# smoorjani/matrix-multiplication

Hardware: AMD Instinct MI355X
Metric: SpMM GFLOP/s, CSR(1M,0.01%) x dense(256) (higher is better)
Workload: dtype f32

## Files before the change

### include/mi_spmm.h

```cpp
#ifndef MI_SPMM_H_
#define MI_SPMM_H_

#include <stddef.h>
#include <stdint.h>

#ifdef __cplusplus
extern "C" {
#endif

#define MI_SPMM_ABI_VERSION 1

typedef void* mi_stream_t;

enum {
  MI_OK = 0,
  MI_EINVAL = -1,
  MI_ERANGE = -2,
  MI_EHIP = -3,
  MI_ENOMEM = -4,
  MI_EUNSORTED = -5
};

int mi_spmm_abi_version(void);
const char* mi_status_string(int status);
// ... 31 lines not shown
  MI_SPMM_GROUP_VEC4 = 4,
  MI_SPMM_GROUP_SCALAR = 5,
  MI_SPMM_WAVE_ROW_VL = 6,
  MI_SPMM_PANELS_2 = 7,
  MI_SPMM_PANELS_3 = 8,
  MI_SPMM_PANELS_4 = 9,
  MI_SPMM_PANELS_5 = 10,
  MI_SPMM_PANELS_6 = 11,
  MI_SPMM_PANELS_8 = 12,
  MI_SPMM_GROUP_VEC2 = 13,
  MI_SPMM_COLTILE = 14,
  MI_SPMM_COLTILE_PANELS = 15,
  MI_SPMM_NARROW = 16,
  MI_SPMM_SLAB = 17,
  MI_SPMM_LDS_B = 18,
  MI_SPMM_GROUP_PANELS_2 = 19,
  MI_SPMM_GROUP_PANELS_3 = 20,
  MI_SPMM_GROUP_PANELS_4 = 21,
  MI_SPMM_GROUP_PANELS_6 = 22,
  MI_SPMM_GROUP_PANELS_8 = 23,
  MI_SPMM_GROUP_VEC4U = 24,
  MI_SPMM_VARIANT_COUNT = 25
};
int mi_spmm_ldsb_set_form(int form);
int mi_spmm_csr_f32_variant(int variant, const int32_t* rowptr, const int32_t* col,
                            const float* val, int64_t nnz, int32_t M, int32_t K,
                            int32_t N, const float* B, int64_t ldb, float* C,
                            int64_t ldc, mi_stream_t stream);
int mi_spmm_csr_ex_variant_f32(int variant, const int32_t* rowptr, const int32_t* col, const float* val,
                               int64_t nnz, int32_t M, int32_t K, int32_t N, const float* B, int64_t ldb,
                               const float* bias, float* C, int64_t ldc, int long_rows, void* workspace,
                               size_t workspace_bytes, mi_stream_t stream);

int mi_spmm_csr_f32_plan(int64_t nnz, int32_t M, int32_t K, int32_t N, const float* B,
                         int64_t ldb, const float* C, int64_t ldc);
int mi_spmm_variant_launches(int variant);
const char* mi_spmm_variant_name(int variant);

typedef struct mi_spmm_schedule mi_spmm_schedule_t;
size_t mi_spmm_schedule_workspace_bytes(int32_t M);
#define MI_SCHEDULE_HOST_INTS 512
int mi_spmm_schedule_begin(const int32_t* rowptr, const int32_t* col, int32_t M, int32_t K, int64_t nnz, int32_t N,
                           int32_t* order, int32_t* order_locality, void* workspace, size_t workspace_bytes,
                           int32_t* host_out, mi_stream_t stream);
int mi_spmm_schedule_finish(const int32_t* host_out, int32_t* order, int32_t* order_locality, int32_t M, int32_t K, int64_t nnz,
                            int32_t N, mi_spmm_schedule_t** out);
int mi_spmm_schedule_create(const int32_t* rowptr, const int32_t* col, int32_t M, int32_t K, int64_t nnz, int32_t N,
                            int32_t* order, void* workspace, size_t workspace_bytes, mi_stream_t stream,
                            mi_spmm_schedule_t** out);
int mi_spmm_schedule_destroy(mi_spmm_schedule_t* schedule);
#define MI_SPMM_SCHEDULE_INFO_LEN 12
int mi_spmm_schedule_info(const mi_spmm_schedule_t* schedule, int64_t* info);
int mi_spmm_schedule_set_heavy(mi_spmm_schedule_t* schedule, int32_t heavy_len, int use_side_stream);
int mi_spmm_csr_scheduled_f32(const mi_spmm_schedule_t* schedule, int variant, const int32_t* rowptr, const int32_t* col,
                              const float* val, int64_t nnz, int32_t M, int32_t K, int32_t N, const float* B, int64_t ldb,
                              const float* bias, float* C, int64_t ldc, int long_rows, void* workspace,
                              size_t workspace_bytes, mi_stream_t stream);
int mi_spmm_csr_colmajor_sched_f32(const mi_spmm_schedule_t* schedule, const int32_t* rowptr, const int32_t* col,
                                   const float* val, int64_t nnz, int32_t M, int32_t K, int32_t N, const float* B,
                                   int64_t ldb, float* C, int64_t ldc, int long_rows, void* long_rows_workspace,
                                   size_t long_rows_workspace_bytes, void* workspace, size_t workspace_bytes,
                                   mi_stream_t stream);

int mi_spmm_csr_batched_f32(const int32_t* rowptr, const int32_t* col,
                            const float* val, int64_t nnz_total, int32_t batch,
                            int32_t M, int32_t K, int32_t N, const float* B,
                            int64_t ldb, int64_t strideB, float* C, int64_t ldc,
                            int64_t strideC, mi_stream_t stream);
int mi_spmm_csr_batched_perm_f32(const int32_t* rowptr, const int32_t* col, const float* val,
                                 const int32_t* perm, int64_t nnz_total, int32_t batch, int32_t M,
                                 int32_t K, int32_t N, const float* B, int64_t ldb, int64_t strideB,
                                 float* C, int64_t ldc, int64_t strideC, mi_stream_t stream);
int mi_spmm_csr_batched_variant_f32(int variant, const int32_t* rowptr, const int32_t* col,
                                    const float* val, int64_t nnz_total, int32_t batch,
                                    int32_t M, int32_t K, int32_t N, const float* B,
                                    int64_t ldb, int64_t strideB, float* C, int64_t ldc,
                                    int64_t strideC, mi_stream_t stream);
int mi_spmm_csr_batched_at_f32(const int32_t* rowptr, const int32_t* col, const float* val, int64_t nnz_total,
                               int32_t batch, int32_t M, int32_t K, int32_t N, const float* X, int64_t ldx,
                               int64_t strideX, float* Y, int64_t ldy, int64_t strideY, mi_stream_t stream);
int mi_batched_csr_narrow_i64(const int64_t* crow, const int64_t* col, int32_t batch, int32_t M, int64_t per_item,
                              int32_t* offsets, int32_t* columns, mi_stream_t stream);
int mi_spmm_csr_batched_f32_plan(int64_t nnz_total, int32_t batch, int32_t M, int32_t K, int32_t N,
                                 const float* B, int64_t ldb, int64_t strideB, const float* C,
                                 int64_t ldc, int64_t strideC);

size_t mi_spmm_colmajor_workspace_bytes(int32_t M, int32_t K, int32_t N);
int mi_spmm_csr_colmajor_f32(const int32_t* rowptr, const int32_t* col,
                             const float* val, int64_t nnz, int32_t M, int32_t K,
                             int32_t N, const float* B, int64_t ldb, float* C,
                             int64_t ldc, void* workspace, size_t workspace_bytes,
                             mi_stream_t stream);
int mi_spmm_colmajor_native_form(int64_t nnz, int32_t M, int32_t K, int32_t N, const float* B,
                                 int64_t ldb, const float* C, int64_t ldc);
int mi_spmm_colmajor_form(int64_t nnz, int32_t M, int32_t K, int32_t N, const float* B, int64_t ldb,
                          const float* C, int64_t ldc, const void* workspace);
int mi_spmm_csr_colmajor_ex_f32(const int32_t* rowptr, const int32_t* col,
                                const float* val, int64_t nnz, int32_t M, int32_t K,
                                int32_t N, const float* B, int64_t ldb, float* C,
                                int64_t ldc, int long_rows, void* long_rows_workspace,
                                size_t long_rows_workspace_bytes, void* workspace,
                                size_t workspace_bytes, mi_stream_t stream);

int mi_gemm_f32(int transa, int transb, int32_t m, int32_t n, int32_t k,
                const float* A, int64_t lda, int64_t strideA, const float* B,
                int64_t ldb, int64_t strideB, float* C, int64_t ldc,
// ... 137 lines not shown
```

### matrix-multiplication_amd/csrc/custom_mm.cpp

```cpp
#include <torch/extension.h>

#include <c10/hip/HIPGuard.h>
#include <c10/hip/HIPStream.h>

#include <array>
#include <cstdlib>
#include <initializer_list>
#include <map>
#include <memory>
#include <mutex>
#include <string>
#include <tuple>
#include <unordered_map>
#include <utility>

#include "mi_spmm.h"

namespace {
#include "custom_mm_helpers.inc"
#include "custom_mm_reference.inc"
#include "custom_mm_extras.inc"
#include "custom_mm_inspect.inc"
#include "custom_mm_reduce.inc"

// ... 32 lines not shown
  m.def("cusparse_mmul", &cusparse_mmul, "cuSPARSE Torch Matrix Multiplication");

  m.def("dummy_kernel", &dummy_kernel_launch, "Launch dummy kernel.");
  m.def("naive_spmm", &naive_spmm, "A naive implementation of Sparse Matrix Multiplication");

  m.def("tiledspmm_inspect_csr", &tiledspmm_inspect_csr, "Inspect function for TiledSpMM with CSR input");
  m.def("tiledspmm_inspect_coo", &tiledspmm_inspect_coo, "Inspect function for TiledSpMM with COO input");
  m.def("tiledspmm_mm", &tiledspmm_mm, "MM function for TiledSpMM");
  m.def("tiledspmm_clean", &tiledspmm_clean, "Cleanup function for TiledSpMM");

  m.def("cusparse_inspect", &cusparse_inspect, "Inspect function for CuSPARSE with CSR input");
  m.def("cusparse_mmul_opt", &cusparse_mmul_opt, "MM function for CuSPARSE");
  m.def("cusparse_clean", &cusparse_clean, "Cleanup function for CuSPARSE");
  m.def("cusparse_mmul_opt_t", &cusparse_mmul_opt_t, "column-major product with the cached transpose: C = A^T B");
  m.def("tiledspmm_mm_t", &tiledspmm_mm_t, "column-major product with the cached transpose: C = A^T B");
  m.def("inspect_info", &inspect_info, "what an inspector handle holds (layer, tiled)");

  m.def("dense_to_csr", &dense_to_csr, "Device dense -> batched CSR (values, columns, offsets)");
  m.def("dense_row_offsets", &dense_row_offsets, "Device dense -> row offsets [batch, rows+1] only (no host sync)");
  m.def("dense_to_csr_fill", &dense_to_csr_fill, "(values, columns) for the offsets of dense_row_offsets");
  m.def("naive_spmm_batched", &naive_spmm_batched, "Batched CSR x dense in one launch");
  m.def("csr_transpose", &csr_transpose, "Device CSR transpose (values, columns, offsets)");
  m.def("csr_transpose_batched", &csr_transpose_batched, "Batched device CSR transpose (values, columns, offsets [batch, cols+1])");
  m.def("csr_transpose_in_lds", [](int64_t nnz, int64_t batch, int64_t rows, int64_t cols) {
          return rows <= INT32_MAX && cols <= INT32_MAX && batch <= INT32_MAX &&
                 mi_csr_transpose_batched_in_lds(nnz, (int32_t)batch, (int32_t)rows, (int32_t)cols) == 1;
        }, "does csr_transpose_batched run the one-workgroup-per-item LDS plan on this batch (cheap: transpose per backward)");
  m.def("sddmm", &sddmm, "Sampled dense-dense product on a CSR pattern");
  m.def("cublas_bmm_pair", &cublas_bmm_pair,
        "dA = dC.B and dB = dC^T.A in one launch that reads dC once; (dC, B, A, dA, dB) -> launched?");
  m.def("sddmm_batched", &sddmm_batched,
        "SDDMM on a batched CSR pattern into out[nnz]; False (nothing launched) if the LDS-resident form does not take it");
  m.def("gather_perm", &gather_perm, "values[perm] (int32 perm) as a new tensor");
  m.def("naive_spmm_batched_perm", &naive_spmm_batched_perm,
        "naive_spmm_batched with entry p's value = A_values[perm[p]]; False (nothing launched) if the plan takes no permutation");
  m.def("naive_spmm_batched_at", &naive_spmm_batched_at,
        "C[i] = A[i]^T X[i] for a batched CSR A without transposing it; False (nothing launched) if the shape is not covered");
  m.def("batched_csr_narrow", &batched_csr_narrow,
        "(int32 offsets [batch, rows+1] with the items' bases, int32 columns) of int64 crow [batch, rows+1] / col [batch, per_item]");
  m.def("naive_spmm_dense", &naive_spmm_dense,
        "A·B with A dense, zeros skipped in the kernel; False if the shape is not covered");
  m.def("naive_spmm_dense_bias", &naive_spmm_dense_bias, "as naive_spmm_dense, + bias in the epilogue");
  m.def("nonfinite_flag", &nonfinite_flag, "int32[1] device tensor: 1 if the tensor holds an inf / nan (nothing read back)");
  m.def("naive_spmm_dense_gated", &naive_spmm_dense_gated,
        "naive_spmm_dense as a launch that runs only when flag[0] != 0 on the device; (A, B, C, flag, dry_run) -> covered?");
  m.def("cublas_mmul_bias", &cublas_mmul_bias, "op(A) op(B) + bias, fused epilogue");
  m.def("column_sums", &column_sums, "sum over rows of a 2-d tensor (bias gradient)");
  m.def("naive_spmm_bias", &naive_spmm_bias, "CSR x dense + bias, fused epilogue");
  m.def("naive_spmm_ex", &naive_spmm_ex, "naive_spmm with the long-row rule pinned (-1 auto, 0 none, 1 split)");
  m.def("naive_spmm_bias_ex", &naive_spmm_bias_ex, "naive_spmm_bias with the long-row rule pinned (-1 auto, 0 none, 1 split)");
  m.def("spmm_plan", &spmm_plan, "(variant, kernel name, launches, splits_long_rows) of the AUTO plan");
  m.def("validate_csr", &validate_csr, "opt-in check of CSR contents (offsets monotone, columns in range); raises");
  py::class_<PySchedule, std::shared_ptr<PySchedule>>(m, "SpmmSchedule")
      .def("info", &PySchedule::info, "rows, heavy_rows, heavy_length, classes, longest_at_least, side_stream, active, locality_order, window spans, nnz, width")
      .def("set_heavy", &PySchedule::set_heavy, py::arg("heavy_length"), py::arg("side_stream") = true,
           "another heavy length / the heavy launch in line (tests, A/B)")
      .def_readonly("order", &PySchedule::order, "int32 [rows] on the device: slot -> row, rows by descending length class");
  m.def("spmm_schedule", &spmm_schedule, py::arg("A_offsets"), py::arg("nnzA"), py::arg("A_rows"), py::arg("N"),
        py::arg("A_columns") = py::none(), py::arg("A_cols") = 0,
        "Inspector: the row schedule of a CSR matrix (offsets, nnz, rows, dense width; with the columns: also tries the locality order)");
  m.def("naive_spmm_scheduled", &naive_spmm_scheduled, py::arg("schedule"), py::arg("A_values"), py::arg("A_columns"),
        py::arg("A_offsets"), py::arg("nnzA"), py::arg("A_rows"), py::arg("A_cols"), py::arg("B"), py::arg("C"),
        py::arg("bias") = py::none(), py::arg("long_rows") = -1, py::arg("variant") = 0,
        "naive_spmm on a row schedule: the same bits, rows handed to waves longest first");
  m.def("auto_schedule_stats", &auto_schedule_stats, "the automatic row schedules of the plain entry points: enabled, entries, pending, active, inactive, built");
  m.def("auto_schedule_clear", &auto_schedule_clear, "forget every automatic row schedule");
  m.def("ipc_export", &ipc_export, "(handle bytes, offset, allocation bytes) of a device buffer, for a peer process to map");
  m.def("ipc_open", &ipc_open, "a peer's exported buffer as a tensor (valid until ipc_close of the handle)");
  m.def("ipc_close", &ipc_close, "drop one open of a peer handle");
  m.def("ipc_open_count", []() { return mi_ipc_open_count(); }, "peer mappings not yet closed in this process");
  m.def("long_row_threshold", &long_row_threshold, "rows with more non-zeros are 'long' (split rule)");
  m.def("naive_spmm_reduce", &naive_spmm_reduce, py::arg("A_values"), py::arg("A_columns"), py::arg("A_offsets"),
        py::arg("nnzA"), py::arg("A_rows"), py::arg("A_cols"), py::arg("B"), py::arg("C"), py::arg("reduce"),
        py::arg("arg") = py::none(),
        "CSR x dense with reduce = sum / mean / amax / amin (torch.sparse.mm); amax / amin write the selected entries to arg");
  m.def("spmm_rows_divide", &spmm_rows_divide, "out = in / (entries of the row), per row (mean and its gradient)");
  m.def("spmm_reduce_grad_val", &spmm_reduce_grad_val, "amax / amin: gradient of A's stored values from the forward's arg");
  m.def("spmm_reduce_grad_b", &spmm_reduce_grad_b, "amax / amin: gradient of B on A^T's pattern and permutation");
  py::module_::import("atexit").attr("register")(py::cpp_function([]() {
    auto_schedule_clear();
    std::lock_guard<std::mutex> lock(g_registry_mutex);
    g_cusparse_layers.clear();
    g_tiled_layers.clear();
  }));
}
```

### matrix-multiplication_amd/csrc/custom_mm_reference.inc

```

torch::Tensor cublas_mmul(torch::Tensor A, torch::Tensor B, torch::Tensor C, bool transa,
                          bool transb) {
  return gemm_impl(A, B, C, 0, transa, transb, "cublas_mmul");
}

torch::Tensor cublas_bmm(torch::Tensor A, torch::Tensor B, torch::Tensor C, int dim, bool transa,
                         bool transb) {
  if (dim == 3) return gemm_impl(A, B, C, 1, transa, transb, "cublas_bmm");
  if (dim == 4) return gemm_impl(A, B, C, 2, transa, transb, "cublas_bmm");
  if (dim == 2) return cublas_mmul(A, B, C, transa, transb);
  throw std::invalid_argument("Invalid dim argument.");
}


struct StreamWorkspace {
  torch::Tensor buf;
};
std::mutex g_stream_ws_mutex;
std::map<std::pair<int, mi_stream_t>, StreamWorkspace> g_stream_ws;

bool stream_is_capturing(mi_stream_t stream) {
  hipStreamCaptureStatus status = hipStreamCaptureStatusNone;
  if (hipStreamIsCapturing(static_cast<hipStream_t>(stream), &status) != hipSuccess) {
    (void)hipGetLastError();
    return true;
  }
  return status != hipStreamCaptureStatusNone;
}

torch::Tensor zeroed_stream_workspace(const torch::Device& dev, mi_stream_t stream, size_t bytes) {
  std::lock_guard<std::mutex> lock(g_stream_ws_mutex);
  const auto key = std::make_pair((int)dev.index(), stream);
  if (g_stream_ws.size() >= 64 && g_stream_ws.find(key) == g_stream_ws.end())
    g_stream_ws.clear();
  StreamWorkspace& w = g_stream_ws[key];
  if (!w.buf.defined() || (size_t)w.buf.numel() < bytes) {
    const int64_t cap = (int64_t)(bytes + bytes / 2 + 4096);
    w.buf = torch::empty({cap}, torch::dtype(torch::kUInt8).device(dev));
    w.buf.narrow(0, 0, 16).zero_();
  }
  return w.buf;
}

void drop_stream_workspace(const torch::Device& dev, mi_stream_t stream) {
  std::lock_guard<std::mutex> lock(g_stream_ws_mutex);
  g_stream_ws.erase(std::make_pair((int)dev.index(), stream));
}

std::array<int64_t, MI_SPMM_SCHEDULE_INFO_LEN> schedule_info(const mi_spmm_schedule_t* sc, const char* what) {
  std::array<int64_t, MI_SPMM_SCHEDULE_INFO_LEN> v{};
  check_status(mi_spmm_schedule_info(sc, v.data()), what);
  return v;
}

struct PySchedule {
  torch::Tensor order;
  torch::Tensor order_keep;
  mi_spmm_schedule_t* sc = nullptr;
  int64_t rows = 0, nnz = 0;
  torch::Tensor long_ws;
  int64_t long_ws_width = -1;
  int64_t long_rows = -1;
  ~PySchedule() { mi_spmm_schedule_destroy(sc); }
  py::dict info() const {
    const auto v = schedule_info(sc, "SpmmSchedule.info");
    py::dict d;
    d["rows"] = v[0];
    d["heavy_rows"] = v[1];
    d["heavy_length"] = v[2];
    d["classes"] = v[3];
    d["longest_at_least"] = v[4];
    d["side_stream"] = (v[5] & 1) != 0;
    d["active"] = (v[5] & 2) != 0;
    d["locality_order"] = (v[5] & 4) != 0;
    d["window_span_natural"] = v[8] < 0 ? -1.0 : v[8] / 1000.0;
    d["window_span_scheduled"] = v[9] < 0 ? -1.0 : v[9] / 1000.0;
    d["row_span"] = v[10] < 0 ? -1.0 : v[10] / 1000.0;
    d["long_rows"] = long_rows;
    d["nnz"] = v[6];
    d["width"] = v[7];
    d["long_rows_prepared"] = long_ws.defined();
    return d;
  }
  void set_heavy(int64_t heavy_len, bool side_stream) {
    check_status(mi_spmm_schedule_set_heavy(sc, (int32_t)heavy_len, side_stream ? 1 : 0), "SpmmSchedule.set_heavy");
  }
};

struct AutoEntry {
  int seen = 0;
  bool pending = false, failed = false, active = false;
  std::shared_ptr<PySchedule> sched;
  torch::Tensor order_buf, ws, host;
  hipEvent_t ev = nullptr;
  uint64_t stamp = 0;
};
using AutoKey = std::tuple<int, mi_stream_t, const void*, const void*, int64_t, int64_t>;
std::mutex g_auto_mutex;
std::map<AutoKey, AutoEntry> g_auto;
uint64_t g_auto_clock = 0;
int64_t g_auto_built = 0;

bool auto_schedule_enabled() {
  static const bool on = []() {
    const char* e = std::getenv("MI_AUTO_SCHEDULE");
    return !(e != nullptr && e[0] == '0');
  }();
  return on;
}

void auto_drop(AutoEntry& e) {
  if (e.ev != nullptr) (void)hipEventDestroy(e.ev);
  e.ev = nullptr;
}

std::shared_ptr<PySchedule> auto_schedule(const torch::Tensor& A_offsets, const torch::Tensor& A_columns, int64_t nnzA,
                                          int64_t A_rows, int64_t A_cols, int64_t N, mi_stream_t stream) {
  if (!auto_schedule_enabled() || nnzA < (1 << 14) || A_rows < 1024 || A_cols > INT32_MAX || stream_is_capturing(stream)) return nullptr;
  std::lock_guard<std::mutex> lock(g_auto_mutex);
  const AutoKey key{(int)A_offsets.device().index(), stream, A_offsets.data_ptr(), A_columns.data_ptr(), A_rows, nnzA};
  AutoEntry& e = g_auto[key];
  e.seen++;
  e.stamp = ++g_auto_clock;
  if (e.sched) return e.active ? e.sched : nullptr;
  if (e.failed) return nullptr;
  if (e.pending) {
    if (e.ev == nullptr) return nullptr;
    const hipError_t q = hipEventQuery(e.ev);
    if (q == hipErrorNotReady) {
      (void)hipGetLastError();
      return nullptr;
    }
    e.pending = false;
    auto_drop(e);
    if (q != hipSuccess) {
      e.failed = true;
      return nullptr;
    }
    auto out = std::make_shared<PySchedule>();
    int32_t* order = e.order_buf.data_ptr<int32_t>();
    if (mi_spmm_schedule_finish(e.host.data_ptr<int32_t>(), order, order + A_rows, (int32_t)A_rows, (int32_t)A_cols, nnzA, (int32_t)N,
                                &out->sc) != MI_OK) {
      e.failed = true;
      return nullptr;
    }
    const auto v = schedule_info(out->sc, "auto_schedule");
    out->rows = A_rows;
    out->nnz = nnzA;
    out->order_keep = e.order_buf;
    out->order = (v[5] & 4) ? e.order_buf.narrow(0, A_rows, A_rows) : e.order_buf.narrow(0, 0, A_rows);
    if (!(v[5] & 2)) out->order_keep = out->order = torch::Tensor();
    e.order_buf = e.ws = e.host = torch::Tensor();
    e.sched = out;
    e.active = (v[5] & 2) != 0;
    g_auto_built++;
    return e.active ? e.sched : nullptr;
  }
  if (e.seen == 2) {
    try {
      auto iopt = torch::dtype(torch::kInt32).device(A_offsets.device());
      e.order_buf = torch::empty({2 * A_rows}, iopt);
      e.ws = byte_workspace(A_offsets.device(), mi_spmm_schedule_workspace_bytes((int32_t)A_rows));
      e.host = torch::empty({MI_SCHEDULE_HOST_INTS}, torch::dtype(torch::kInt32).pinned_memory(true));
      e.pending = true;
    } catch (...) {
      e.failed = true;
      e.order_buf = e.ws = e.host = torch::Tensor();
    }
  }
  if (g_auto.size() > 16) {
    auto victim = g_auto.end();
    for (auto it = g_auto.begin(); it != g_auto.end(); ++it)
      if (!it->second.pending && &it->second != &e && (victim == g_auto.end() || it->second.stamp < victim->second.stamp)) victim = it;
    if (victim != g_auto.end()) {
      auto_drop(victim->second);
      g_auto.erase(victim);
    }
  }
  return nullptr;
}

void auto_schedule_launch(const torch::Tensor& A_offsets, const torch::Tensor& A_columns, int64_t nnzA, int64_t A_rows,
                          int64_t A_cols, int64_t N, mi_stream_t stream) {
  if (!auto_schedule_enabled()) return;
  std::lock_guard<std::mutex> lock(g_auto_mutex);
  auto it = g_auto.find(AutoKey{(int)A_offsets.device().index(), stream, A_offsets.data_ptr(), A_columns.data_ptr(), A_rows, nnzA});
  if (it == g_auto.end()) return;
  AutoEntry& e = it->second;
  if (!e.pending || e.ev != nullptr || !e.order_buf.defined()) return;
  int32_t* order = e.order_buf.data_ptr<int32_t>();
  const int st = mi_spmm_schedule_begin(A_offsets.data_ptr<int32_t>(), A_columns.data_ptr<int32_t>(), (int32_t)A_rows, (int32_t)A_cols,
                                        nnzA, (int32_t)N, order, order + A_rows, e.ws.data_ptr(), (size_t)e.ws.numel(),
                                        e.host.data_ptr<int32_t>(), stream);
  bool ok = st == MI_OK && hipEventCreateWithFlags(&e.ev, hipEventDisableTiming) == hipSuccess &&
            hipEventRecord(e.ev, static_cast<hipStream_t>(stream)) == hipSuccess;
  if (!ok) {
    auto_drop(e);
    e.pending = false;
    e.failed = true;
    e.order_buf = e.ws = e.host = torch::Tensor();
  }
}

py::dict auto_schedule_stats() {
  std::lock_guard<std::mutex> lock(g_auto_mutex);
  int64_t pending = 0, active = 0, inactive = 0;
  for (auto& kv : g_auto) {
// ... 250 lines not shown
```

### matrix-multiplication_amd/csrc/spmm_csr.hip

```cpp
#include "spmm_device.h"
#include "spmm_internal.h"

namespace {

using mi::LongArg;
using mi::Shape;

template <int T, int U>
__global__ __launch_bounds__(256) void spmm_wave_row_kernel(
    const int* __restrict__ rowptr, const int* __restrict__ col,
    const float* __restrict__ val, const float* __restrict__ B, float* __restrict__ C,
    int M, long ldb, long ldc, long strideB, long strideC, const float* __restrict__ bias,
    LongArg la) {
  const int lane = threadIdx.x & 63;
  const int wave = __builtin_amdgcn_readfirstlane(threadIdx.x >> 6);
  const long slot = (long)blockIdx.x * 4 + wave;
  if (slot >= (la.order ? la.nslots : M)) return;
  const long row = la.order ? la.order[slot] : slot;
  const long item = blockIdx.y;
  const int* rp = rowptr + item * ((long)M + 1);
  const float* Bl = B + item * strideB + lane * 4;
  float* Cl = C + item * strideC + row * ldc + lane * 4;

  int p = rp[row];
// ... 501 lines not shown
      return dispatch_group<4>(rowptr, col, val, B, C, M, N, ldb, ldc, strideB, strideC, batch, bias, la, s);
    }
    case MI_SPMM_NARROW: {
      if (N >= 4) return MI_EINVAL;
      const long blocks = ((long)M + 3) / 4;
      if (blocks > 0x7fffffffL) return MI_ERANGE;
      hipLaunchKernelGGL(spmm_narrow_kernel, dim3((unsigned)blocks, (unsigned)batch), dim3(256), 0, s, rowptr, col,
                         val, B, C, M, N, ldb, ldc, strideB, strideC, bias);
      return mi::check_launch();
    }
    default:
      return MI_EINVAL;
  }
#undef MI_WAVE
}

bool variant_takes_order(int variant) {
  switch (variant) {
    case MI_SPMM_WAVE_ROW_U4: case MI_SPMM_WAVE_ROW_U8: case MI_SPMM_WAVE_ROW_U16:
    case MI_SPMM_GROUP_VEC4: case MI_SPMM_GROUP_VEC2: case MI_SPMM_GROUP_SCALAR: case MI_SPMM_GROUP_VEC4U:
    case MI_SPMM_PANELS_2: case MI_SPMM_PANELS_3: case MI_SPMM_PANELS_4: case MI_SPMM_PANELS_5: case MI_SPMM_PANELS_6:
    case MI_SPMM_PANELS_8:
    case MI_SPMM_GROUP_PANELS_2: case MI_SPMM_GROUP_PANELS_3: case MI_SPMM_GROUP_PANELS_4: case MI_SPMM_GROUP_PANELS_6:
    case MI_SPMM_GROUP_PANELS_8:
      return true;
    default:
      return false;
  }
}

}

namespace mi {

int spmm_dispatch(int variant, const int32_t* rowptr, const int32_t* col, const float* val,
                  int64_t nnz, int32_t batch, int32_t M, int32_t K, int32_t N, const float* B,
                  int64_t ldb, int64_t strideB, float* C, int64_t ldc, int64_t strideC,
                  const float* bias, void* workspace, size_t workspace_bytes, hipStream_t s,
                  int long_mode, const RowSchedule* sched) {
  if (M < 0 || K < 0 || N < 0 || nnz < 0 || batch < 0) return MI_EINVAL;
  if (variant < 0 || variant >= MI_SPMM_VARIANT_COUNT) return MI_EINVAL;
  if (long_mode < MI_LONG_ROWS_AUTO || long_mode > MI_LONG_ROWS_AUTO_ZEROED) return MI_EINVAL;
  if (nnz > 0x7fffffffLL) return MI_ERANGE;
  if (batch > 65535) return MI_ERANGE;
  if (M == 0 || N == 0 || batch == 0) return MI_OK;
  if (!rowptr || !C) return MI_EINVAL;
  if (nnz > 0 && (!col || !val || !B)) return MI_EINVAL;
  if (ldb < N || ldc < N) return MI_EINVAL;
  if (sched != nullptr && (sched->rows != M || sched->order == nullptr || batch != 1)) return MI_EINVAL;

  Shape sh = classify(N, ldb, ldc, strideB, strideC, B, C);
  if (bias && !mi::aligned16(bias)) sh.vec4_ok = sh.wave_ok = false;
  if (bias && (reinterpret_cast<uintptr_t>(bias) & 7u)) sh.vec2_ok = false;
  if (variant == MI_SPMM_AUTO) variant = choose_variant(sh, nnz, batch, M, K, N, ldb);
  if (sched != nullptr && (!sched->active || !variant_takes_order(variant))) sched = nullptr;

  const bool pinned_split = long_mode == MI_LONG_ROWS_SPLIT || long_mode == MI_LONG_ROWS_PREPARED;
  const bool split = workspace != nullptr && batch == 1 && nnz > kLongRow && variant != MI_SPMM_NARROW &&
                     long_mode != MI_LONG_ROWS_NONE && (variant != MI_SPMM_SLAB || pinned_split);
  int* ws = static_cast<int*>(workspace);
  const LongWs lw = long_ws_layout(nnz, N);
  LongArg la = {0x7fffffff, 0, 0, 0, nullptr, nullptr, nullptr, 0};
  const bool prepared = long_mode == MI_LONG_ROWS_PREPARED;
  const bool panel_plan = (variant >= MI_SPMM_PANELS_2 && variant <= MI_SPMM_PANELS_8) ||
                          (variant >= MI_SPMM_GROUP_PANELS_2 && variant <= MI_SPMM_GROUP_PANELS_8);
  const double b_bytes_all = (double)K * (double)ldb * 4.0;
  if (panel_plan && batch == 1 && nnz > 0 && b_bytes_all < 768.0 * 1048576.0 && workspace != nullptr && workspace_bytes >= lw.bytes &&
      (reinterpret_cast<uintptr_t>(workspace) & 15u) == 0) {
    int* verdicts = reinterpret_cast<int*>(static_cast<char*>(workspace) + lw.adapt_off);
    const int st = launch_locality_probe(rowptr, col, M, ldb, b_bytes_all, verdicts, sched != nullptr ? sched->order : nullptr, s);
    if (st != MI_OK) return st;
    la.adapt = verdicts;
  }
  if (split) {
    if (workspace_bytes < lw.bytes) return MI_ENOMEM;
    if ((reinterpret_cast<uintptr_t>(workspace) & 15u) != 0) return MI_EINVAL;
    la.thresh = kLongRow;
    la.cap_e = (int)lw.cap_e, la.cap_s = (int)lw.cap_s, la.cap_p = (int)lw.cap_p;
    if (!prepared) {
      if (long_mode != MI_LONG_ROWS_AUTO_ZEROED) MI_HIP_TRY(hipMemsetAsync(ws, 0, 16, s));
      if (variant == MI_SPMM_SLAB || variant == MI_SPMM_LDS_B) {
        LongArg fl = la;
        fl.ws = ws;
        const int st = launch_find_long_rows(rowptr, M, fl, s);
        if (st != MI_OK) return st;
      } else {
        la.ws = ws;
      }
    }
  }
  int st = MI_OK;
  bool long_rows_done = false;
  if (sched == nullptr) {
    st = launch_variant(variant, sh, rowptr, col, val, nnz, batch, M, K, N, B, ldb, strideB, C, ldc, strideC, bias, la, s);
  } else {
    const int heavy_slots = sched->heavy < 0 ? 0 : (sched->heavy > M ? M : sched->heavy);
    const int heavy = N >= 4 ? heavy_slots : 0;
    LongArg lh = la, lr = la;
    lh.order = sched->order, lh.nslots = heavy;
    lh.adapt = nullptr;
    const bool early_list = split && !prepared && heavy_slots > 0 && la.ws != nullptr;
    const bool fork = sched->side != nullptr && sched->fork != nullptr && sched->join != nullptr &&
                      (heavy > 0 || (split && prepared) || early_list);
    if (early_list) {
      st = launch_find_long_rows(rowptr, M, la, s);
      if (st != MI_OK) return st;
    }
    hipStream_t rest = s;
    if (fork) {
      MI_HIP_TRY(hipEventRecord(sched->fork, s));
      MI_HIP_TRY(hipStreamWaitEvent(sched->side, sched->fork, 0));
      rest = sched->side;
    }
    if (early_list) {
      lh.ws = nullptr;
      st = launch_staged_rows(ws, lw, false, lh, rowptr, col, val, B, C, N, ldb, ldc, bias, s);
      if (st != MI_OK) return st;
      MI_HIP_TRY(hipMemsetAsync(ws, 0, 16, s));
      long_rows_done = true;
      lr.ws = nullptr;
    } else if (split && prepared && heavy > 0) {
      st = launch_staged_rows(ws, lw, false, lh, rowptr, col, val, B, C, N, ldb, ldc, bias, s);
      if (st != MI_OK) return st;
      long_rows_done = true;
    } else if (split && prepared) {
      st = launch_long_rows(ws, lw, rowptr, col, val, B, C, N, ldb, ldc, bias, false, s);
      if (st != MI_OK) return st;
      long_rows_done = true;
    } else if (heavy > 0) {
      st = launch_heavy_rows(rowptr, col, val, M, N, B, ldb, C, ldc, bias, lh, s);
      if (st != MI_OK) return st;
    }
    lr.order = sched->order + heavy, lr.nslots = M - heavy;
    st = launch_variant(variant, sh, rowptr, col, val, nnz, batch, M, K, N, B, ldb, strideB, C, ldc, strideC, bias, lr, rest);
    if (fork) {
      MI_HIP_TRY(hipEventRecord(sched->join, sched->side));
      MI_HIP_TRY(hipStreamWaitEvent(s, sched->join, 0));
    }
  }
  if (st != MI_OK || !split || long_rows_done) return st;
  return launch_long_rows(ws, lw, rowptr, col, val, B, C, N, ldb, ldc, bias, !prepared, s);
}

}

namespace {
// ... 119 lines not shown
```

### matrix-multiplication_amd/csrc/spmm_internal.h

```cpp
#ifndef MI_SPMM_INTERNAL_H_
#define MI_SPMM_INTERNAL_H_

#include "mi_common.h"

namespace mi {

constexpr int kLongRowThreshold = 8192;
constexpr int kAdaptVerdicts = 16;

struct LongArg {
  int thresh;
  int cap_e, cap_s, cap_p;
  int* ws;
  const int* adapt;
  const int* order;
  int nslots;
};

struct LongWs {
  long cap_e, cap_s, cap_p;
  size_t owner_off, partial_off, bytes;
  size_t adapt_off;
};
LongWs long_ws_layout(int64_t nnz, int32_t N);
int launch_find_long_rows(const int32_t* rowptr, int32_t M, const LongArg& la, hipStream_t s);
int launch_long_rows(int* ws, const LongWs& lw, const int32_t* rowptr, const int32_t* col, const float* val, const float* B,
                     float* C, int32_t N, int64_t ldb, int64_t ldc, const float* bias, bool reset, hipStream_t s);
int launch_long_rows_staged(int* ws, const LongWs& lw, const int32_t* rowptr, const int32_t* col, const float* val,
                            const float* B, float* C, int32_t N, int64_t ldb, int64_t ldc, const float* bias, bool reset,
                            hipStream_t s);

int launch_locality_probe(const int32_t* rowptr, const int32_t* col, int32_t M, int64_t ldb, double b_bytes, int* verdicts,
                          const int32_t* order, hipStream_t s);
int launch_panels(int panels, const int* rowptr, const int* col, const float* val, const float* B, float* C, int M, int K,
                  int N, long ldb, long ldc, const float* bias, LongArg la, hipStream_t s);
int launch_coltile_panels(int panels, const int* rowptr, const int* col, const float* val, const float* B, float* C, int M,
                          int K, int N, long ldb, long ldc, const float* bias, LongArg la, hipStream_t s);
int group_panel_count(int variant);
int launch_group_panels(int panels, const int* rowptr, const int* col, const float* val, const float* B, float* C, int M,
                        int K, int N, long ldb, long ldc, const float* bias, LongArg la, hipStream_t s);

int launch_heavy_rows(const int32_t* rowptr, const int32_t* col, const float* val, int32_t M, int32_t N, const float* B,
                      int64_t ldb, float* C, int64_t ldc, const float* bias, LongArg la, hipStream_t s);
int launch_staged_rows(int* ws, const LongWs& lw, bool reset, const LongArg& heavy, const int32_t* rowptr, const int32_t* col,
                       const float* val, const float* B, float* C, int32_t N, int64_t ldb, int64_t ldc, const float* bias,
                       hipStream_t s);

struct Shape {
  bool vec4_ok, vec2_ok, wave_ok;
};
Shape classify(int32_t N, int64_t ldb, int64_t ldc, int64_t strideB, int64_t strideC, const float* B, const float* C);
int choose_variant(const Shape& sh, int64_t nnz, int32_t batch, int32_t M, int32_t K, int32_t N, int64_t ldb);
int coltile_width(int32_t M, int32_t K, int32_t N, int64_t ldb);
int coltile_panels(int32_t M, int32_t K, int32_t N, int64_t ldb, int64_t nnz);

struct RowSchedule {
  const int32_t* order;
  int32_t rows;
  int32_t heavy;
  int32_t heavy_len;
  bool active;
  hipStream_t side;
  hipEvent_t fork, join;
};
int spmm_dispatch(int variant, const int32_t* rowptr, const int32_t* col, const float* val, int64_t nnz, int32_t batch,
                  int32_t M, int32_t K, int32_t N, const float* B, int64_t ldb, int64_t strideB, float* C, int64_t ldc,
                  int64_t strideC, const float* bias, void* workspace, size_t workspace_bytes, hipStream_t s,
                  int long_mode = MI_LONG_ROWS_AUTO, const RowSchedule* sched = nullptr);

}

#endif
```

### matrix-multiplication_amd/csrc/spmm_sched.hip

```cpp
#include <map>
#include <mutex>
#include <new>

#include "spmm_device.h"
#include "spmm_internal.h"

namespace {

constexpr int kClasses = 256;
constexpr int kTileRows = 2048;
constexpr int kWindows = 16;
constexpr int kHeavyRowsMost = 128;
static_assert(kClasses + 1 + 2 * 3 * kWindows < MI_SCHEDULE_HOST_INTS, "the class table and both window statistics fit host_out");

__host__ __device__ __forceinline__ int length_class(int len) {
  if (len < 32) return len < 0 ? 0 : len;
  const int e = 31 - __builtin_clz((unsigned)len);
  return 32 + (e - 5) * 8 + ((len >> (e - 3)) & 7);
}
int class_floor(int c) {
  if (c < 32) return c;
  const int e = 5 + (c - 32) / 8, m = (c - 32) % 8;
  return (1 << e) + (m << (e - 3));
}
// ... 246 lines not shown
    if (e == hipSuccess) {
      hipLaunchKernelGGL(sched_window_stats_kernel, dim3(kWindows), dim3(256), 0, s, rowptr, col, M, K, (const int*)order_locality,
                         stats + 3 * kWindows);
      e = hipGetLastError();
    }
    if (e == hipSuccess)
      e = hipMemcpyAsync(host_out + kClasses + 1, stats, 2 * 3 * kWindows * sizeof(int), hipMemcpyDeviceToHost, s);
  }
  if (e == hipSuccess) e = counting_pass<kKeyClass>(rowptr, col, M, K, nullptr, order, table, start, s);
  if (e == hipSuccess) e = hipMemcpyAsync(host_out, start, (kClasses + 1) * sizeof(int), hipMemcpyDeviceToHost, s);
  if (e != hipSuccess) return mi::record_hip_error(e);
  host_out[MI_SCHEDULE_HOST_INTS - 1] = try_locality ? 1 : 0;
  return MI_OK;
}

int mi_spmm_schedule_finish(const int32_t* host_out, int32_t* order, int32_t* order_locality, int32_t M, int32_t K, int64_t nnz,
                            int32_t N, mi_spmm_schedule_t** out) {
  if (!out) return MI_EINVAL;
  *out = nullptr;
  if (!host_out || M < 0 || K < 0 || nnz < 0 || N < 0 || (M > 0 && !order)) return MI_EINVAL;
  mi_spmm_schedule* sc = new (std::nothrow) mi_spmm_schedule();
  if (!sc) return MI_ENOMEM;
  sc->rs = mi::RowSchedule{order, M, 0, 0, true, nullptr, nullptr, nullptr};
  sc->nnz = nnz;
  sc->n_width = N;
  sc->locality = false;
  sc->span_natural = sc->span_scheduled = sc->span_row = -1;
  for (int b = 0; b <= kClasses; ++b) sc->start[b] = M > 0 ? host_out[b] : 0;
  if (M > 0 && host_out[MI_SCHEDULE_HOST_INTS - 1] == 1 && order_locality != nullptr && K > 0) {
    const int32_t* h_stats = host_out + kClasses + 1;
    double nat = 0, neu = 0, row = 0;
    int wn = 0;
    for (int w = 0; w < kWindows; ++w) {
      if (h_stats[3 * w + 2] == 0 && h_stats[3 * (kWindows + w) + 2] == 0) continue;
      nat += h_stats[3 * w], neu += h_stats[3 * (kWindows + w)], row += h_stats[3 * w + 1];
      ++wn;
    }
    if (wn > 0) {
      sc->span_natural = (int32_t)(1000.0 * nat / wn / kClasses);
      sc->span_scheduled = (int32_t)(1000.0 * neu / wn / kClasses);
      sc->span_row = (int32_t)(1000.0 * row / wn / K);
      sc->locality = sc->span_natural > 400 && 2 * sc->span_scheduled < sc->span_natural;
      if (sc->locality) sc->rs.order = order_locality;
    }
  }
  sc->longest = 0, sc->classes = 0;
  for (int b = kClasses - 1; b >= 0; --b) {
    if (sc->start[b + 1] > sc->start[b]) {
      sc->classes++;
      sc->longest = class_floor(kClasses - 1 - b);
    }
  }
  set_heavy(sc, heavy_length_for(nnz, M), true);
  if (sc->rs.active && (sc->rs.heavy > 0 || sc->longest + sc->longest / 8 + 1 > mi::kLongRowThreshold)) {
    const int st = ensure_side_stream(sc);
    if (st != MI_OK) {
      mi_spmm_schedule_destroy(sc);
      return st;
    }
  }
  *out = sc;
  return MI_OK;
}

int mi_spmm_schedule_create(const int32_t* rowptr, const int32_t* col, int32_t M, int32_t K, int64_t nnz, int32_t N,
                            int32_t* order, void* workspace, size_t workspace_bytes, mi_stream_t stream,
                            mi_spmm_schedule_t** out) {
  if (!out) return MI_EINVAL;
  *out = nullptr;
  int32_t host[MI_SCHEDULE_HOST_INTS];
  int32_t* order_locality = (col != nullptr && order != nullptr) ? order + (M > 0 ? M : 0) : nullptr;
  int st = mi_spmm_schedule_begin(rowptr, col, M, K, nnz, N, order, order_locality, workspace, workspace_bytes, host, stream);
  if (st != MI_OK) return st;
  const hipError_t e = hipStreamSynchronize(static_cast<hipStream_t>(stream));
  if (e != hipSuccess) return mi::record_hip_error(e);
  return mi_spmm_schedule_finish(host, order, order_locality, M, K, nnz, N, out);
}

int mi_spmm_schedule_destroy(mi_spmm_schedule_t* sc) {
  if (!sc) return MI_OK;
  if (sc->rs.fork) (void)hipEventDestroy(sc->rs.fork);
  if (sc->rs.join) (void)hipEventDestroy(sc->rs.join);
  delete sc;
  return MI_OK;
}

int mi_spmm_schedule_info(const mi_spmm_schedule_t* sc, int64_t* info) {
  if (!sc || !info) return MI_EINVAL;
  const int64_t v[MI_SPMM_SCHEDULE_INFO_LEN] = {
      sc->rs.rows, sc->rs.heavy, sc->rs.heavy_len, sc->classes, sc->longest,
      (sc->rs.side != nullptr ? 1 : 0) | (sc->rs.active ? 2 : 0) | (sc->locality ? 4 : 0),
      sc->nnz, sc->n_width, sc->span_natural, sc->span_scheduled, sc->span_row, 0};
  for (int i = 0; i < MI_SPMM_SCHEDULE_INFO_LEN; ++i) info[i] = v[i];
  return MI_OK;
}

int mi_spmm_schedule_set_heavy(mi_spmm_schedule_t* sc, int32_t heavy_len, int use_side_stream) {
  if (!sc || heavy_len < 0) return MI_EINVAL;
  set_heavy(sc, heavy_len, false);
  sc->rs.active = true;
  if (!use_side_stream && sc->rs.side) {
    sc->rs.side = nullptr;
  }
  if (use_side_stream) return ensure_side_stream(sc);
  return MI_OK;
}

int mi_spmm_csr_scheduled_f32(const mi_spmm_schedule_t* sc, int variant, const int32_t* rowptr, const int32_t* col,
                              const float* val, int64_t nnz, int32_t M, int32_t K, int32_t N, const float* B, int64_t ldb,
                              const float* bias, float* C, int64_t ldc, int long_rows, void* workspace,
                              size_t workspace_bytes, mi_stream_t stream) {
  if (!sc) return MI_EINVAL;
  if (long_rows == MI_LONG_ROWS_SPLIT && workspace == nullptr && nnz > mi::kLongRowThreshold) return MI_EINVAL;
  return mi::spmm_dispatch(variant, rowptr, col, val, nnz, 1, M, K, N, B, ldb, 0, C, ldc, 0, bias, workspace, workspace_bytes,
                           static_cast<hipStream_t>(stream), long_rows, &sc->rs);
}

}
```

Measured before the change: 3573.

## Add L2-windowed row-rounds SpMM kernel for N=256 with large dense B

Adds a new kernel in which each wave owns 48 rows and advances through B in column-index windows of 512 rows. It gathers only nonzeros whose column falls below the current window, using global_load_lds into a double-buffered LDS ring. The goal is to keep the working set of B in L2 when B exceeds about 768 MiB, so gathers hit cache instead of HBM. It is enabled through the schedule only for AUTO plans with N=256, wave-aligned shapes, panel variants and no stream capture. The cost is extra ballot and readlane overhead and lower per-row parallelism.

```diff
diff --git a/include/mi_spmm.h b/include/mi_spmm.h
--- a/include/mi_spmm.h
+++ b/include/mi_spmm.h
@@ -107,6 +107,7 @@
 #define MI_SPMM_SCHEDULE_INFO_LEN 12
 int mi_spmm_schedule_info(const mi_spmm_schedule_t* schedule, int64_t* info);
 int mi_spmm_schedule_set_heavy(mi_spmm_schedule_t* schedule, int32_t heavy_len, int use_side_stream);
+int mi_spmm_schedule_set_rounds(mi_spmm_schedule_t* schedule, int on);
 int mi_spmm_csr_scheduled_f32(const mi_spmm_schedule_t* schedule, int variant, const int32_t* rowptr, const int32_t* col,
                               const float* val, int64_t nnz, int32_t M, int32_t K, int32_t N, const float* B, int64_t ldb,
                               const float* bias, float* C, int64_t ldc, int long_rows, void* workspace,
diff --git a/matrix-multiplication_amd/csrc/custom_mm.cpp b/matrix-multiplication_amd/csrc/custom_mm.cpp
--- a/matrix-multiplication_amd/csrc/custom_mm.cpp
+++ b/matrix-multiplication_amd/csrc/custom_mm.cpp
@@ -108,9 +108,11 @@
   m.def("spmm_plan", &spmm_plan, "(variant, kernel name, launches, splits_long_rows) of the AUTO plan");
   m.def("validate_csr", &validate_csr, "opt-in check of CSR contents (offsets monotone, columns in range); raises");
   py::class_<PySchedule, std::shared_ptr<PySchedule>>(m, "SpmmSchedule")
-      .def("info", &PySchedule::info, "rows, heavy_rows, heavy_length, classes, longest_at_least, side_stream, active, locality_order, window spans, nnz, width")
+      .def("info", &PySchedule::info, "rows, heavy_rows, heavy_length, classes, longest_at_least, side_stream, active, locality_order, rounds, window spans, nnz, width")
       .def("set_heavy", &PySchedule::set_heavy, py::arg("heavy_length"), py::arg("side_stream") = true,
            "another heavy length / the heavy launch in line (tests, A/B)")
+      .def("set_rounds", &PySchedule::set_rounds, py::arg("on"),
+           "row rounds on (every AUTO product of N = 256 with 16-byte rows) or off (tests, A/B)")
       .def_readonly("order", &PySchedule::order, "int32 [rows] on the device: slot -> row, rows by descending length class");
   m.def("spmm_schedule", &spmm_schedule, py::arg("A_offsets"), py::arg("nnzA"), py::arg("A_rows"), py::arg("N"),
         py::arg("A_columns") = py::none(), py::arg("A_cols") = 0,
diff --git a/matrix-multiplication_amd/csrc/custom_mm_reference.inc b/matrix-multiplication_amd/csrc/custom_mm_reference.inc
--- a/matrix-multiplication_amd/csrc/custom_mm_reference.inc
+++ b/matrix-multiplication_amd/csrc/custom_mm_reference.inc
@@ -73,6 +73,7 @@
     d["side_stream"] = (v[5] & 1) != 0;
     d["active"] = (v[5] & 2) != 0;
     d["locality_order"] = (v[5] & 4) != 0;
+    d["rounds"] = (v[5] & 8) != 0;
     d["window_span_natural"] = v[8] < 0 ? -1.0 : v[8] / 1000.0;
     d["window_span_scheduled"] = v[9] < 0 ? -1.0 : v[9] / 1000.0;
     d["row_span"] = v[10] < 0 ? -1.0 : v[10] / 1000.0;
@@ -85,6 +86,7 @@
   void set_heavy(int64_t heavy_len, bool side_stream) {
     check_status(mi_spmm_schedule_set_heavy(sc, (int32_t)heavy_len, side_stream ? 1 : 0), "SpmmSchedule.set_heavy");
   }
+  void set_rounds(bool on) { check_status(mi_spmm_schedule_set_rounds(sc, on ? 1 : 0), "SpmmSchedule.set_rounds"); }
 };
 
 struct AutoEntry {
@@ -149,10 +151,11 @@
     out->nnz = nnzA;
     out->order_keep = e.order_buf;
     out->order = (v[5] & 4) ? e.order_buf.narrow(0, A_rows, A_rows) : e.order_buf.narrow(0, 0, A_rows);
-    if (!(v[5] & 2)) out->order_keep = out->order = torch::Tensor();
+    const bool used = (v[5] & (2 | 8)) != 0;
+    if (!used) out->order_keep = out->order = torch::Tensor();
     e.order_buf = e.ws = e.host = torch::Tensor();
     e.sched = out;
-    e.active = (v[5] & 2) != 0;
+    e.active = used;
     g_auto_built++;
     return e.active ? e.sched : nullptr;
   }
diff --git a/matrix-multiplication_amd/csrc/spmm_csr.hip b/matrix-multiplication_amd/csrc/spmm_csr.hip
--- a/matrix-multiplication_amd/csrc/spmm_csr.hip
+++ b/matrix-multiplication_amd/csrc/spmm_csr.hip
@@ -577,8 +577,16 @@
   Shape sh = classify(N, ldb, ldc, strideB, strideC, B, C);
   if (bias && !mi::aligned16(bias)) sh.vec4_ok = sh.wave_ok = false;
   if (bias && (reinterpret_cast<uintptr_t>(bias) & 7u)) sh.vec2_ok = false;
+  const bool auto_plan = variant == MI_SPMM_AUTO;
   if (variant == MI_SPMM_AUTO) variant = choose_variant(sh, nnz, batch, M, K, N, ldb);
-  if (sched != nullptr && (!sched->active || !variant_takes_order(variant))) sched = nullptr;
+  const double b_bytes_all = (double)K * (double)ldb * 4.0;
+  bool rounds = false;
+  if (sched != nullptr && sched->rounds != 0 && auto_plan && batch == 1 && N == 256 && sh.wave_ok && nnz > 0) {
+    const bool ic_panels = variant >= MI_SPMM_PANELS_2 && variant <= MI_SPMM_PANELS_8 && b_bytes_all >= 768.0 * 1048576.0;
+    hipStreamCaptureStatus cap = hipStreamCaptureStatusNone;
+    rounds = (sched->rounds == 2 || ic_panels) && hipStreamIsCapturing(s, &cap) == hipSuccess && cap == hipStreamCaptureStatusNone;
+  }
+  if (sched != nullptr && !rounds && (!sched->active || !variant_takes_order(variant))) sched = nullptr;
 
   const bool pinned_split = long_mode == MI_LONG_ROWS_SPLIT || long_mode == MI_LONG_ROWS_PREPARED;
   const bool split = workspace != nullptr && batch == 1 && nnz > kLongRow && variant != MI_SPMM_NARROW &&
@@ -589,8 +597,7 @@
   const bool prepared = long_mode == MI_LONG_ROWS_PREPARED;
   const bool panel_plan = (variant >= MI_SPMM_PANELS_2 && variant <= MI_SPMM_PANELS_8) ||
                           (variant >= MI_SPMM_GROUP_PANELS_2 && variant <= MI_SPMM_GROUP_PANELS_8);
-  const double b_bytes_all = (double)K * (double)ldb * 4.0;
-  if (panel_plan && batch == 1 && nnz > 0 && b_bytes_all < 768.0 * 1048576.0 && workspace != nullptr && workspace_bytes >= lw.bytes &&
+  if (panel_plan && !rounds && batch == 1 && nnz > 0 && b_bytes_all < 768.0 * 1048576.0 && workspace != nullptr && workspace_bytes >= lw.bytes &&
       (reinterpret_cast<uintptr_t>(workspace) & 15u) == 0) {
     int* verdicts = reinterpret_cast<int*>(static_cast<char*>(workspace) + lw.adapt_off);
     const int st = launch_locality_probe(rowptr, col, M, ldb, b_bytes_all, verdicts, sched != nullptr ? sched->order : nullptr, s);
@@ -616,7 +623,11 @@
   }
   int st = MI_OK;
   bool long_rows_done = false;
-  if (sched == nullptr) {
+  if (rounds) {
+    LongArg lr = la;
+    lr.order = sched->order, lr.nslots = M;
+    st = launch_l2_rounds(rowptr, col, val, B, C, M, K, ldb, ldc, bias, lr, s);
+  } else if (sched == nullptr) {
     st = launch_variant(variant, sh, rowptr, col, val, nnz, batch, M, K, N, B, ldb, strideB, C, ldc, strideC, bias, la, s);
   } else {
     const int heavy_slots = sched->heavy < 0 ? 0 : (sched->heavy > M ? M : sched->heavy);
diff --git a/matrix-multiplication_amd/csrc/spmm_internal.h b/matrix-multiplication_amd/csrc/spmm_internal.h
--- a/matrix-multiplication_amd/csrc/spmm_internal.h
+++ b/matrix-multiplication_amd/csrc/spmm_internal.h
@@ -40,6 +40,9 @@
 int launch_group_panels(int panels, const int* rowptr, const int* col, const float* val, const float* B, float* C, int M,
                         int K, int N, long ldb, long ldc, const float* bias, LongArg la, hipStream_t s);
 
+int launch_l2_rounds(const int32_t* rowptr, const int32_t* col, const float* val, const float* B, float* C, int32_t M, int32_t K,
+                     int64_t ldb, int64_t ldc, const float* bias, LongArg la, hipStream_t s);
+
 int launch_heavy_rows(const int32_t* rowptr, const int32_t* col, const float* val, int32_t M, int32_t N, const float* B,
                       int64_t ldb, float* C, int64_t ldc, const float* bias, LongArg la, hipStream_t s);
 int launch_staged_rows(int* ws, const LongWs& lw, bool reset, const LongArg& heavy, const int32_t* rowptr, const int32_t* col,
@@ -62,6 +65,7 @@
   bool active;
   hipStream_t side;
   hipEvent_t fork, join;
+  int rounds = 0;
 };
 int spmm_dispatch(int variant, const int32_t* rowptr, const int32_t* col, const float* val, int64_t nnz, int32_t batch,
                   int32_t M, int32_t K, int32_t N, const float* B, int64_t ldb, int64_t strideB, float* C, int64_t ldc,
diff --git a/matrix-multiplication_amd/csrc/spmm_rounds.hip b/matrix-multiplication_amd/csrc/spmm_rounds.hip
--- /dev/null
+++ b/matrix-multiplication_amd/csrc/spmm_rounds.hip
@@ -0,0 +1,188 @@
+#include "spmm_device.h"
+#include "spmm_internal.h"
+
+#include <cstdlib>
+
+namespace {
+
+using mi::LongArg;
+
+constexpr int kRoundsWin = 8;
+constexpr int kRoundsStepRows = 512;
+
+typedef __attribute__((address_space(3))) void lds_void;
+
+__device__ __forceinline__ void wait_vmem_at_most(int n) {
+#define MI_VM(k) \
+  case k: asm volatile("s_waitcnt vmcnt(" #k ")" ::: "memory"); break;
+  switch (n) {
+    MI_VM(0) MI_VM(1) MI_VM(2) MI_VM(3) MI_VM(4) MI_VM(5) MI_VM(6) MI_VM(7) MI_VM(8)
+    MI_VM(9) MI_VM(10) MI_VM(11) MI_VM(12) MI_VM(13) MI_VM(14) MI_VM(15)
+    default: asm volatile("s_waitcnt vmcnt(16)" ::: "memory"); break;
+  }
+#undef MI_VM
+}
+
+template <int S, int WAVES, int P>
+__global__ __launch_bounds__(64 * WAVES, WAVES / 4) void spmm_l2_rounds_kernel(
+    const int* __restrict__ rowptr, const int* __restrict__ col, const float* __restrict__ val, const float* __restrict__ B,
+    float* __restrict__ C, int K, long ldb, long ldc, const float* __restrict__ bias, long nslots, long blk_base, long blk_count,
+    LongArg la) {
+  static_assert(S <= 64 && P <= 16, "one lane per slot; the wait covers 16 gathers");
+  __shared__ f32x4 s_ring[WAVES][2][P][64];
+  const int lane = threadIdx.x & 63;
+  const int w = __builtin_amdgcn_readfirstlane(threadIdx.x >> 6);
+  const float* Bl = B + lane * 4;
+  const long nblk = (nslots + S - 1) / S;
+  const long blk_end = blk_base + blk_count < nblk ? blk_base + blk_count : nblk;
+  f32x4 b4 = {0.f, 0.f, 0.f, 0.f};
+  if (bias) b4 = *reinterpret_cast<const f32x4*>(bias + lane * 4);
+
+  for (long blk = blk_base + (long)blockIdx.x * WAVES + w; blk < blk_end; blk += (long)gridDim.x * WAVES) {
+    const long slot = blk * S + lane;
+    int row = 0, cur = 0, end = 0;
+    bool own = false;
+    if (lane < S && slot < nslots) {
+      row = la.order ? la.order[slot] : (int)slot;
+      cur = rowptr[row];
+      end = rowptr[row + 1];
+      own = true;
+      if (end - cur > la.thresh) {
+        long_list_append(la, row, end - cur);
+        end = cur;
+        own = false;
+      }
+    }
+    const unsigned long long own_mask = __ballot(own);
+
+    int wc[kRoundsWin];
+    float wv[kRoundsWin];
+    int have = 0;
+    auto refill = [&]() {
+#pragma unroll
+      for (int i = 0; i < kRoundsWin; ++i) {
+        const int idx = cur + i;
+        const bool in = idx < end;
+        wc[i] = in ? col[idx] : 0;
+        wv[i] = in ? val[idx] : 0.f;
+      }
+      have = end - cur < kRoundsWin ? end - cur : kRoundsWin;
+    };
+    refill();
+
+    f32x4 acc[S];
+#pragma unroll
+    for (int s = 0; s < S; ++s) acc[s] = f32x4{0.f, 0.f, 0.f, 0.f};
+    int rmax = kIntMin;
+    int hi = 0;
+    int ph = 0;
+    unsigned long long m_old = 0ull;
+    float v_old = 0.f;
+
+    auto consume = [&](int h, unsigned long long m, float v) {
+      f32x4(*half)[64] = s_ring[w][h];
+      int k = 0;
+#pragma unroll
+      for (int s = 0; s < S; ++s) {
+        if ((m >> s) & 1ull) {
+          const float vs = __builtin_bit_cast(float, __builtin_amdgcn_readlane(__builtin_bit_cast(int, v), s));
+          acc[s] = fma4(vs, half[k][lane], acc[s]);
+          ++k;
+        }
+      }
+      asm volatile("s_waitcnt lgkmcnt(0)" ::: "memory");
+    };
+
+    for (;;) {
+      if (__ballot(have == 0 && cur < end) != 0ull) refill();
+      const bool live = cur < end;
+      if (__ballot(live) == 0ull) break;
+      const int c = wc[0];
+      const float v = wv[0];
+      const int pm = c > rmax ? c : rmax;
+      bool all = hi >= K;
+      unsigned long long m = __ballot(live && (all || pm < hi));
+      while (!all && __builtin_popcountll(m) < P) {
+        hi = hi < K - kRoundsStepRows ? hi + kRoundsStepRows : K;
+        all = hi >= K;
+        m = __ballot(live && (all || pm < hi));
+      }
+      int n = __builtin_popcountll(m);
+      if (n > P) {
+        unsigned long long rest = m;
+#pragma unroll
+        for (int i = 0; i < P; ++i) rest &= rest - 1ull;
+        m ^= rest;
+        n = P;
+      }
+      unsigned long long t = m;
+      for (int k = 0; k < n; ++k) {
+        const int s = __builtin_ctzll(t);
+        t &= t - 1ull;
+        const int cs = __builtin_amdgcn_readlane(c, s);
+        __builtin_amdgcn_global_load_lds(Bl + (long)cs * ldb, (lds_void*)&s_ring[w][ph][k][0], 16, 0, 0);
+      }
+      if ((m >> lane) & 1ull) {
+        rmax = pm;
+        ++cur;
+        --have;
+#pragma unroll
+        for (int i = 0; i + 1 < kRoundsWin; ++i) {
+          wc[i] = wc[i + 1];
+          wv[i] = wv[i + 1];
+        }
+      }
+      wait_vmem_at_most(n);
+      consume(ph ^ 1, m_old, v_old);
+      m_old = m;
+      v_old = v;
+      ph ^= 1;
+    }
+    wait_vmem_at_most(0);
+    consume(ph ^ 1, m_old, v_old);
+
+#pragma unroll
+    for (int s = 0; s < S; ++s) {
+      if ((own_mask >> s) & 1ull) {
+        const long r = __builtin_amdgcn_readlane(row, s);
+        __builtin_nontemporal_store(bias ? acc[s] + b4 : acc[s], reinterpret_cast<f32x4*>(C + r * ldc + lane * 4));
+      }
+    }
+  }
+}
+
+int cu_count() {
+  int dev = 0, n = 0;
+  if (hipGetDevice(&dev) != hipSuccess || hipDeviceGetAttribute(&n, hipDeviceAttributeMultiprocessorCount, dev) != hipSuccess ||
+      n <= 0)
+    n = 256;
+  return n;
+}
+
+}
+
+namespace mi {
+
+int launch_l2_rounds(const int32_t* rowptr, const int32_t* col, const float* val, const float* B, float* C, int32_t M, int32_t K,
+                     int64_t ldb, int64_t ldc, const float* bias, LongArg la, hipStream_t s) {
+  constexpr int kS = 48, kWaves = 8, kP = 8;
+  const long nslots = la.order ? la.nslots : M;
+  if (nslots <= 0) return MI_OK;
+  static const int cus = cu_count();
+  const long blocks_needed = (nslots + (long)kS * kWaves - 1) / ((long)kS * kWaves);
+  const unsigned grid = (unsigned)(blocks_needed < cus ? blocks_needed : cus);
+  const long nblk = (nslots + kS - 1) / kS;
+  static const bool per_round = [] { const char* e = std::getenv("MI_ROUNDS_LAUNCH"); return e != nullptr && e[0] == '1'; }();
+  if (!per_round) {
+    hipLaunchKernelGGL((spmm_l2_rounds_kernel<kS, kWaves, kP>), dim3(grid), dim3(64 * kWaves), 0, s, rowptr, col, val, B, C, K,
+                       (long)ldb, (long)ldc, bias, nslots, 0L, nblk, la);
+    return check_launch();
+  }
+  const long per = (long)grid * kWaves;
+  for (long b0 = 0; b0 < nblk; b0 += per)
+    hipLaunchKernelGGL((spmm_l2_rounds_kernel<kS, kWaves, kP>), dim3(grid), dim3(64 * kWaves), 0, s, rowptr, col, val, B, C, K,
+                       (long)ldb, (long)ldc, bias, nslots, b0, per, la);
+  return check_launch();
+}
+
+}
diff --git a/matrix-multiplication_amd/csrc/spmm_sched.hip b/matrix-multiplication_amd/csrc/spmm_sched.hip
--- a/matrix-multiplication_amd/csrc/spmm_sched.hip
+++ b/matrix-multiplication_amd/csrc/spmm_sched.hip
@@ -322,6 +322,7 @@
     }
   }
   set_heavy(sc, heavy_length_for(nnz, M), true);
+  sc->rs.rounds = (N == 256 && M > 0 && nnz > 0 && (double)K * 256.0 * 4.0 >= 768.0 * 1048576.0) ? 1 : 0;
   if (sc->rs.active && (sc->rs.heavy > 0 || sc->longest + sc->longest / 8 + 1 > mi::kLongRowThreshold)) {
     const int st = ensure_side_stream(sc);
     if (st != MI_OK) {
@@ -359,7 +360,7 @@
   if (!sc || !info) return MI_EINVAL;
   const int64_t v[MI_SPMM_SCHEDULE_INFO_LEN] = {
       sc->rs.rows, sc->rs.heavy, sc->rs.heavy_len, sc->classes, sc->longest,
-      (sc->rs.side != nullptr ? 1 : 0) | (sc->rs.active ? 2 : 0) | (sc->locality ? 4 : 0),
+      (sc->rs.side != nullptr ? 1 : 0) | (sc->rs.active ? 2 : 0) | (sc->locality ? 4 : 0) | (sc->rs.rounds != 0 ? 8 : 0),
       sc->nnz, sc->n_width, sc->span_natural, sc->span_scheduled, sc->span_row, 0};
   for (int i = 0; i < MI_SPMM_SCHEDULE_INFO_LEN; ++i) info[i] = v[i];
   return MI_OK;
@@ -373,6 +374,12 @@
     sc->rs.side = nullptr;
   }
   if (use_side_stream) return ensure_side_stream(sc);
+  return MI_OK;
+}
+
+int mi_spmm_schedule_set_rounds(mi_spmm_schedule_t* sc, int on) {
+  if (!sc) return MI_EINVAL;
+  sc->rs.rounds = on ? 2 : 0;
   return MI_OK;
 }
 
```

After: 3075 (median of 2 runs). 13.9% lower.
